# k-flouris/cmf

Hardware: AMD Instinct MI355X
Metric: log-density evals/sec (JtJ-cholesky path), MNIST D=784 d=64 bs=512 (higher is better)
Workload: dtype f32 (3x3 tangent convs as bf16x3 split MFMA, fp32 accumulate); 1 GPU; C3: MNIST-shaped (1,28,28) uint8-range + U[0,1) noise, non-square flow d=64, cholesky J^T J log-det + g_ij off-diagonal L1 + reconstruction, eval/no_grad; per_gpu_batch=512, global_batch=512, D=784, latent_dimension=64, parallelism=dp1

## Files before the change

### cmf_amd/_lib.py

```python
import ctypes as C
import os
import threading

_HERE = os.path.dirname(os.path.abspath(__file__))
LIB_PATH = os.path.join(_HERE, "libcmf_amd.so")

F_NONE, F_RELU, F_TANH, F_RAW, F_SELF_RELU, F_RELU_BITS = 0, 1, 2, 3, 4, 5
O_NONE, O_TANH, O_STANH = 0, 1, 2

_fp = C.c_void_p
_ll = C.c_longlong
_i = C.c_int
_f = C.c_float
_d = C.c_double


class ConvTangentArgs(C.Structure):
    _fields_ = [("x", _fp), ("x_np", _ll), ("x_ci", _ll), ("x_px", _ll),
                ("f", _fp), ("f_np", _ll), ("f_ci", _ll), ("f_px", _ll), ("fmode", _i),
                ("w", _fp),
                ("y", _fp), ("y_np", _ll), ("y_co", _ll), ("y_px", _ll),
                ("r", _fp), ("r_np", _ll), ("r_co", _ll), ("r_px", _ll),
                ("np", _i), ("cin", _i), ("cout", _i), ("H", _i), ("W", _i), ("nc", _i), ("taps", _i),
                ("bias", _fp), ("f_group", _i), ("x_sl", _ll), ("y_sl", _ll), ("r_sl", _ll),
                ("fo", _fp), ("fo_np", _ll), ("fo_co", _ll), ("fo_px", _ll), ("fomode", _i),
                ("mask_out", _fp), ("mask_np", _ll), ("amax_in", _fp), ("amax_out", _fp), ("live", _i)]


class ConvPrimalArgs(C.Structure):
    _fields_ = [("x", _fp), ("x_b", _ll), ("x_c", _ll), ("x_px", _ll),
                ("f", _fp), ("f_c", _ll), ("f_px", _ll), ("imode", _i),
                ("w", _fp), ("bias", _fp), ("sw", _fp), ("sb", _fp),
                ("y", _fp), ("y_b", _ll), ("y_c", _ll), ("y_px", _ll),
                ("g", _fp),
                ("r", _fp), ("r_b", _ll), ("r_c", _ll), ("r_px", _ll),
                ("omode", _i),
                ("B", _i), ("cin", _i), ("cout", _i), ("H", _i), ("W", _i), ("taps", _i)]


MLP_MAX_LAYERS = 8
WGRAD_MAX_BATCH = 16
# ... 166 lines not shown
```

### cmf_amd/csrc/conv_tangent.hip

```cpp
#include <type_traits>
#include "common.h"

namespace {

constexpr int CIC = 8;

template <int TAPS, int COT, int PXW>
struct Cfg {
  static constexpr int TW = 2 * PXW;
  static constexpr int TWH = TW + 2;
  static constexpr int PIXH = (TAPS == 9) ? 4 * TWH : 4 * PXW;
  static constexpr int XS_CI = PIXH * 16 + 16;
  static constexpr int WS_CI = (COT % 2) ? COT * 16 : COT * 16 + 16;
  static constexpr int XS_FLOATS = CIC * XS_CI;
  static constexpr int WS_FLOATS = TAPS * CIC * WS_CI;
  static constexpr int NX_ITEMS = CIC * PIXH * 4;
  static constexpr int NXIT = (NX_ITEMS + 255) / 256;
  static constexpr int NW_ITEMS = TAPS * CIC * COT * 4;
  static constexpr int NWIT = (NW_ITEMS + 255) / 256;
};

template <int TAPS, int COT, int PXW>
__global__ __launch_bounds__(256, 2) void conv_tangent_kernel(cmf_conv_tangent_args a, int tiles_x, int ntiles,
                                                                int nslices, int ncog, int cin_pad, int nsub) {
// ... 380 lines not shown

extern "C" int cmf_conv_tangent(const cmf_conv_tangent_args* ap, void* stream) {
  if (!ap) return CMF_EINVAL;
  const cmf_conv_tangent_args& a = *ap;
  if (!a.x || !a.w || !a.y || a.np <= 0 || a.cin <= 0 || a.cout <= 0 || a.H <= 0 || a.W <= 0) return CMF_EINVAL;
  if (a.taps != 1 && a.taps != 9) return CMF_EINVAL;
  if (a.nc <= 0 || a.nc % 16 || a.live) return CMF_EINVAL;
  if (a.fmode < CMF_F_NONE || a.fmode > CMF_F_SELF_RELU) return CMF_EINVAL;
  if (a.fmode != CMF_F_NONE && a.fmode != CMF_F_SELF_RELU && !a.f) return CMF_EINVAL;
  if ((a.x_np | a.x_ci | a.x_px | a.x_sl | a.y_sl | a.r_sl) % 4 || ((uintptr_t)a.x % 16) || ((uintptr_t)a.w % 16)) return CMF_EINVAL;
  if ((a.y_np | a.y_co | a.y_px) % 4 || ((uintptr_t)a.y % 16)) return CMF_EINVAL;
  if (a.r && ((a.r_np | a.r_co | a.r_px) % 4 || ((uintptr_t)a.r % 16))) return CMF_EINVAL;
  if (a.fo && (a.fomode < CMF_F_RELU || a.fomode > CMF_F_SELF_RELU)) return CMF_EINVAL;
  if (a.fo && a.fomode == CMF_F_SELF_RELU && ((a.fo_np | a.fo_co | a.fo_px) % 4 || (uintptr_t)a.fo % 16)) return CMF_EINVAL;
  if (a.mask_out && (a.cout % 16 || a.mask_np < (long long)a.H * a.W * (a.cout / 8))) return CMF_EINVAL;
  const long long HW = (long long)a.H * a.W;
  if (!fits_int((a.cin + 8) * a.x_ci + HW * a.x_px + a.nc) || !fits_int((a.cin + 8) * a.f_ci + HW * a.f_px) ||
      !fits_int((a.cout + 64) * a.y_co + HW * a.y_px + a.nc) || (a.r && !fits_int((a.cout + 64) * a.r_co + HW * a.r_px + a.nc)) ||
      HW > (1 << 24))
    return CMF_ERANGE;
  hipStream_t s = (hipStream_t)stream;
  if (thin_ok(a)) return launch_thin(a, s);
  const bool seven = (a.taps == 9) ? (a.W % 14 == 0) : (HW % 28 == 0 && HW % 32 != 0);
  if (a.taps == 9 && !seven && a.W % 8 == 0 && a.cout % 64 == 0) {
    const long long items8 = (long long)cmf_ceil_div(a.W, 16) * cmf_ceil_div(a.H, 2) * (a.nc / 16) * (a.cout / 64) * a.np;
    if (items8 * 4 <= 128) return launch_cot<9, 4>(a, s);
  }
  if (a.taps == 9) return seven ? launch_cot<9, 7>(a, s) : launch_cot<9, 8>(a, s);
  return seven ? launch_cot<1, 7>(a, s) : launch_cot<1, 8>(a, s);
}
// ... 1 lines not shown
```

### cmf_amd/csrc/conv_tangent_bf16x3.hip

```cpp
#include <cstdlib>
#include <type_traits>
#include "common.h"

#ifdef CMF_DBG_STAMP
__device__ unsigned long long cmf_dbg_stamps[3][64][4];
extern "C" int cmf_debug_read_stamps(void* out) {
  return (int)hipMemcpyFromSymbol(out, HIP_SYMBOL(cmf_dbg_stamps), sizeof(cmf_dbg_stamps));
}
#define STAMP(role, g, k)                                                                        \
  do {                                                                                            \
    if (blockIdx.x == 0 && (g) < 64 && lane == 0 && wave == ((role) == 1 ? 4 : 0)) {                   \
      unsigned long long t_;                                                                      \
      asm volatile("s_memtime %0\n\ts_waitcnt lgkmcnt(0)" : "=s"(t_)::"memory");                  \
      cmf_dbg_stamps[role][g][k] = t_;                                                            \
    }                                                                                             \
  } while (0)
__device__ unsigned long long cmf_dbg_wg_span[1024][2];
extern "C" int cmf_debug_read_wg_span(void* out) {
  return (int)hipMemcpyFromSymbol(out, HIP_SYMBOL(cmf_dbg_wg_span), sizeof(cmf_dbg_wg_span));
}
#define SPAN(k)                                                                                   \
  do {                                                                                            \
    if (lane == 0 && wave == 0 && blockIdx.x < 1024) {                                            \
      unsigned long long t_;                                                                      \
// ... 65 lines not shown
  return __builtin_bit_cast(float, (unsigned)(e + 127) << 23);
}

__device__ __forceinline__ int xslot(int col, int pix) { return (((col & 3) << 2) + (col >> 2) + ((pix & 1) << 2)) & 15; }

template <int COT, int PXW, int MODE, bool F16 = false, bool FRES = false, bool CKB = false>
__global__ __launch_bounds__(512, 2) void conv_tangent_bf16x3_kernel(cmf_conv_tangent_args a, int tiles_x, int ntiles,
                                                                       int nslices, int ncog, int total) {
  static_assert(!CKB || (!F16 && !FRES && (MODE == 1 || MODE == 3)), "checkerboard output: the forward tangent conv with a relu' factor");
  static_assert(!F16 || ((MODE == 2 || MODE == 4) && (COT == 4 || COT == 2)), "the fp16 variant is the primal pass: SELF mode (forward) or 4 (backward)");
  constexpr bool BWD = F16 && MODE == 4;
  static_assert(!BWD || FRES, "the backward form uses the epilogue with tile loads");
  constexpr bool HALF = F16 && COT == 2;
  constexpr int COG = HALF ? 32 : 64;
  static_assert(!FRES || F16, "residual-in-the-epilogue is the fp16 variant's");
  constexpr bool SELF = MODE == 2, RELU = MODE == 1, BITS = MODE == 3;
  constexpr bool PLAIN = !F16 && (MODE == 4 || MODE == 5);
  constexpr bool INPLACE = MODE == 5;
  constexpr bool NOF = SELF || PLAIN || BWD;
  constexpr int NF = NOF ? 0 : BITS ? 1 : 8;
  using C = BCfg<COT, PXW>;
  constexpr int CW = COT / 2, PW = CKB ? C::PW / 2 : C::PW;
  auto tp = [](int p) constexpr { return CKB ? 2 * p : p; };
  auto trow = [&](int p) constexpr { return tp(p) / C::TW; };
  static_assert(COT % 2 == 0, "the co-split wave layout needs an even number of output-channel tiles");
  extern __shared__ __attribute__((aligned(16))) unsigned char smem[];

  const int tid = threadIdx.x, lane = tid & 63;
  const int wave = __builtin_amdgcn_readfirstlane(tid >> 6);
  const bool loader = wave >= 4;
  SPAN(0);
// ... 48 lines not shown
#ifdef CMF_DBG_PRIO
    __builtin_amdgcn_s_setprio(3);
#endif
    const int lt = tid - 256;
    const int x_ci = (int)a.x_ci, x_px = (int)a.x_px, f_ci = (int)a.f_ci, f_px = (int)a.f_px;
    const int q = lt & 3, pix = lt >> 2;
    const int hy = pix / C::TWH, hx = pix % C::TWH;
    const float fc0 = (a.fmode == CMF_F_NONE || a.fmode == CMF_F_TANH || a.fmode == CMF_F_SELF_RELU) ? 1.f : 0.f;
    const float fc1 = (a.fmode == CMF_F_RELU) ? 1.f : 0.f;
    const float fc2 = (a.fmode == CMF_F_RAW) ? 1.f : 0.f;
    const float fc3 = (a.fmode == CMF_F_TANH) ? -1.f : 0.f;
    constexpr bool has_f = !NOF;
    const int fgrp = a.f_group > 1 ? a.f_group : 1;

    typedef int i32x4 __attribute__((ext_vector_type(4)));
    auto make_rsrc = [&](const void* p) {
      const unsigned long long u = reinterpret_cast<unsigned long long>(p);
      i32x4 d;
      d[0] = __builtin_amdgcn_readfirstlane((int)(unsigned)u);
      d[1] = __builtin_amdgcn_readfirstlane((int)((unsigned)(u >> 32) & 0xffffu));
      d[2] = -1;
      d[3] = 0x00020000;
      return d;
    };
    int cur_item = 0, cur_ch = 0;
    i32x4 xrs = make_rsrc(a.x), frs = xrs, wrs = make_rsrc(a.w);
    int xo = 0, fo = 0;
    float okf = 0.f;
    auto set_item = [&](int item) {
      int tile, slice, cog, np;
      decode(item, tile, slice, cog, np);
      const int y0 = C::TH * (tile / tiles_x), x0 = C::TW * (tile % tiles_x);
      xrs = make_rsrc(a.x + (long long)np * a.x_np + (long long)slice * (a.x_sl ? a.x_sl : 16));
      frs = BITS ? make_rsrc(reinterpret_cast<const unsigned char*>(a.f) + (long long)np * a.f_np)
                 : make_rsrc(a.f ? a.f + (long long)(np / fgrp) * a.f_np + (np % fgrp) : a.x);
      const int gy = y0 - 1 + hy, gx = x0 - 1 + hx;
      const bool ok = lt < C::NX_ITEMS && gy >= 0 && gy < a.H && gx >= 0 && gx < a.W;
      const int gpix = gy * a.W + gx;
      okf = ok ? 1.f : 0.f;
      xo = ok ? 4 * (gpix * x_px + q * 4) : 0;
      fo = ok ? (BITS ? gpix * (a.cin / 8) : 4 * (gpix * f_px)) : 0;
    };
    constexpr int NWOFF = COT == 4 ? 1 : C::NWIT;
    int woff[NWOFF];
    if (COT == 4) {
      woff[0] = lt << 4;
    } else {
#pragma unroll
      for (int it = 0; it < NWOFF; ++it) {
        int i = lt + 256 * it;
        i = i < C::NW_ITEMS ? i : C::NW_ITEMS - 1;
        const int rest = i & 63, t = i >> 6;
        const int cot = t % COT, s = (t / COT) % 3, hl = t / (3 * COT);
        woff[it] = (((hl * 3 + s) * 4 + cot) * 64 + rest) << 4;
      }
    }
// ... 24 lines not shown
        if (COT == 4 && it % 3 == 2) {
          asm volatile("s_nop 4\n\tbuffer_load_dwordx4 %0, %1, %2, %3 offen" : "=&v"(wreg[it]) : "v"(vo), "s"(wrs2), "s"(so) : "memory");
          continue;
        }
        asm volatile("s_nop 4\n\tbuffer_load_dwordx4 %0, %1, %2, %3 offen" : "=&v"(wreg[it]) : "v"(vo), "s"(wrs), "s"(so) : "memory");
      }
      if (++wcur_ch == nchunks) {
        wcur_ch = 0;
        if (wcur_item + 1 < n_items) wset_item(++wcur_item);
        else wcur_ch = nchunks - 1;
      }
    };
#pragma unroll
    for (int j = 0; j < 8; ++j) r0.f[j] = r1.f[j] = r2.f[j] = 0.f;

    auto prefetch = [&](Regs& r) {
      const int ch = cur_ch;
      {
        const int s0 = 4 * (ch * 8 + 0) * x_ci, s1 = 4 * (ch * 8 + 1) * x_ci, s2 = 4 * (ch * 8 + 2) * x_ci,
                  s3 = 4 * (ch * 8 + 3) * x_ci, s4 = 4 * (ch * 8 + 4) * x_ci, s5 = 4 * (ch * 8 + 5) * x_ci,
                  s6 = 4 * (ch * 8 + 6) * x_ci, s7 = 4 * (ch * 8 + 7) * x_ci;
        asm volatile(
            "s_nop 4\n\t"
            "buffer_load_dwordx4 %0, %8, %9, %10 offen\n\t"
            "buffer_load_dwordx4 %1, %8, %9, %11 offen\n\t"
            "buffer_load_dwordx4 %2, %8, %9, %12 offen\n\t"
            "buffer_load_dwordx4 %3, %8, %9, %13 offen\n\t"
            "buffer_load_dwordx4 %4, %8, %9, %14 offen\n\t"
            "buffer_load_dwordx4 %5, %8, %9, %15 offen\n\t"
            "buffer_load_dwordx4 %6, %8, %9, %16 offen\n\t"
            "buffer_load_dwordx4 %7, %8, %9, %17 offen"
            : "=&v"(r.x[0]), "=&v"(r.x[1]), "=&v"(r.x[2]), "=&v"(r.x[3]), "=&v"(r.x[4]), "=&v"(r.x[5]), "=&v"(r.x[6]),
              "=&v"(r.x[7])
            : "v"(xo), "s"(xrs), "s"(s0), "s"(s1), "s"(s2), "s"(s3), "s"(s4), "s"(s5), "s"(s6), "s"(s7)
            : "memory");
      }
      if constexpr (BITS) {
        asm volatile("s_nop 4\n\tbuffer_load_ubyte %0, %1, %2, %3 offen" : "=&v"(r.f[0]) : "v"(fo), "s"(frs), "s"(ch) : "memory");
      } else if (has_f) {
        const int s0 = 4 * (ch * 8 + 0) * f_ci, s1 = 4 * (ch * 8 + 1) * f_ci, s2 = 4 * (ch * 8 + 2) * f_ci,
                  s3 = 4 * (ch * 8 + 3) * f_ci, s4 = 4 * (ch * 8 + 4) * f_ci, s5 = 4 * (ch * 8 + 5) * f_ci,
                  s6 = 4 * (ch * 8 + 6) * f_ci, s7 = 4 * (ch * 8 + 7) * f_ci;
        asm volatile(
            "s_nop 4\n\t"
            "buffer_load_dword %0, %8, %9, %10 offen\n\t"
            "buffer_load_dword %1, %8, %9, %11 offen\n\t"
            "buffer_load_dword %2, %8, %9, %12 offen\n\t"
            "buffer_load_dword %3, %8, %9, %13 offen\n\t"
            "buffer_load_dword %4, %8, %9, %14 offen\n\t"
            "buffer_load_dword %5, %8, %9, %15 offen\n\t"
            "buffer_load_dword %6, %8, %9, %16 offen\n\t"
            "buffer_load_dword %7, %8, %9, %17 offen"
            : "=&v"(r.f[0]), "=&v"(r.f[1]), "=&v"(r.f[2]), "=&v"(r.f[3]), "=&v"(r.f[4]), "=&v"(r.f[5]), "=&v"(r.f[6]),
// ... 58 lines not shown
        for (int c = 0; c < 4; ++c) {
          u32x4 h;
#pragma unroll
          for (int jj = 0; jj < 4; ++jj)
            h[jj] = __builtin_amdgcn_perm(__builtin_bit_cast(unsigned, r.x[2 * jj + 1][c]),
                                          __builtin_bit_cast(unsigned, r.x[2 * jj][c]), 0x07060302u);
          const int off = ((pix * 16 + xslot(q * 4 + c, pix)) << 4);
          *reinterpret_cast<u32x4*>(Xh + off) = h;
          *reinterpret_cast<u32x4*>(Xl + off) = h;
        }
#else
        float v[8][4];
#pragma unroll
        for (int j = 0; j < 8; ++j) {
          const float f = r.f[j];
          const float m = NOF ? (F16 ? r.okf * xscale : r.okf) : BITS ? (((__builtin_bit_cast(unsigned, r.f[0]) >> j) & 1u) ? r.okf : 0.f)
                               : RELU ? (f > 0.f ? r.okf : 0.f)
                                              : r.okf * (fc0 + fc1 * (f > 0.f ? 1.f : 0.f) + f * (fc2 + fc3 * f));
#pragma unroll
          for (int c = 0; c < 4; ++c) v[j][c] = (SELF ? fmaxf(r.x[j][c], 0.f) : r.x[j][c]) * m;
        }
#pragma unroll
        for (int c = 0; c < 4; ++c) {
          u32x4 h, l;
#pragma unroll
          for (int jj = 0; jj < 4; ++jj) {
            const float e = v[2 * jj][c], o = v[2 * jj + 1][c];
            if constexpr (F16) {
              unsigned lo_;
              h[jj] = split_f16(e, o, lo_);
              l[jj] = lo_;
            } else {
              const unsigned hb = pack_lo(e, o);
              const float re = e - __builtin_bit_cast(float, hb << 16);
              const float ro = o - __builtin_bit_cast(float, hb & 0xffff0000u);
// ... 15 lines not shown
      for (int it = 0; it < C::NWIT; ++it) {
        const int i = lt + 256 * it;
        if (COT == 4 && it % 3 == 2 && !wquad) continue;
        if (i < C::NW_ITEMS) {
          const int rest = i & 63, t = i >> 6;
          const int cot = t % COT, s = (t / COT) % 3, hl = t / (3 * COT);
          unsigned char* dst = (hl ? Wl : Wh) + ((((s * COT + cot) * 64) + rest) << 4);
          *reinterpret_cast<u32x4*>(dst) = wreg[it];
        }
      }
    };

    if (n_items > 0) {
      set_item(0);
      wset_item(0);
      prefetch(r0);
      prefetch(r1);
      prefetch(r2);
      prefetch_w();
      STAMP2(4, 10, 0);
      asm volatile("s_waitcnt vmcnt(0)" ::: "memory");
      STAMP2(4, 10, 1);
      wait_x(r0);
      commit(r0, 0);
      prefetch_w();
      STAMP2(4, 10, 2);
    }
    __syncthreads();
    auto iter = [&](int g, Regs& freed, Regs& next) {
      STAMP(1, g, 0);
// ... 139 lines not shown
  i32x4 nxt_rrs = r_rsrc(np_, slice_, cog_, n_items > 0);
  auto init_pixel = [&](const Item& it, const i32x4& rrs_in, int p) __attribute__((always_inline)) {
    i32x4 rrs;
#pragma unroll
    for (int i = 0; i < 4; ++i) rrs[i] = __builtin_amdgcn_readfirstlane(rrs_in[i]);
#pragma unroll
    for (int c = 0; c < CW; ++c) {
      const int so = it.rpix + 4 * ((trow(p) * a.W + tp(p) % C::TW + (CKB ? ck_o[trow(p) & 1] : 0)) * r_px + c * 16 * r_co);
      asm volatile("s_nop 4\n\tbuffer_load_dwordx4 %0, %1, %2, %3 offen" : "=v"(acc[p][c]) : "v"(rvoff), "s"(rrs), "s"(so) : "memory");
    }
  };
  unsigned omask[PW];
  const bool use_omask = PLAIN && a.fomode == CMF_F_RELU_BITS;
  constexpr bool inplace = INPLACE;
  auto load_omask = [&](const Item& it) __attribute__((always_inline)) {
    if constexpr (PLAIN) {
      const unsigned long long base = reinterpret_cast<unsigned long long>(a.fo) + (unsigned long long)it.np * a.fo_np +
                                      (unsigned)(it.cog * 8 + cohalf * 4);
      const unsigned lo = __builtin_amdgcn_readfirstlane((int)(unsigned)base);
      const unsigned hi = __builtin_amdgcn_readfirstlane((int)(unsigned)(base >> 32));
      const unsigned long long sb = ((unsigned long long)hi << 32) | lo;
      const int stride = a.cout / 8;
#pragma unroll
      for (int p = 0; p < PW; ++p) {
        const int off = __builtin_amdgcn_readfirstlane((it.pix0 + (p / C::TW) * a.W + p % C::TW) * stride);
        unsigned w;
        asm volatile("s_load_dword %0, %1, %2\n\ts_waitcnt lgkmcnt(0)" : "=&s"(w) : "s"(sb), "s"(off) : "memory");
        omask[p] = use_omask ? w : ~0u;
      }
    }
  };
  auto store_pixel = [&](const Item& it, int p, f32x4 radd0, f32x4 radd1, f32x4 m0 = f32x4{}, f32x4 m1 = f32x4{}) __attribute__((always_inline)) {
    [[maybe_unused]] unsigned mbits = 0;
    [[maybe_unused]] f32x4 vst[CW];
#pragma unroll
    for (int c = 0; c < CW; ++c) {
      f32x4 v = acc[p][c];
      int vo = yvoff;
      if constexpr (PLAIN) {
        const bool on = (omask[p] >> (c * 16 + cl)) & 1u;
        if constexpr (inplace) vo = on ? yvoff : Y_DROP;
        else v = on ? v : f32x4{0.f, 0.f, 0.f, 0.f};
      }
      if constexpr (BWD) {
        v = v * oscale;
        const f32x4 mm = c == 0 ? m0 : m1;
#pragma unroll
        for (int r = 0; r < 4; ++r) v[r] = mm[r] > 0.f ? v[r] : 0.f;
      } else if constexpr (HALF) v = v * oscale + ((it.cog & 1) ? bias_h1 : bias[c]);
      else if constexpr (F16) v = v * oscale + bias[c];
      else v += bias[c];
      if constexpr (FRES) v += c == 0 ? radd0 : radd1;
      __builtin_amdgcn_raw_buffer_store_b128(__builtin_bit_cast(bu32x4, v), cur_yrs, vo,
                                             it.ypix + 4 * ((CKB ? trow(p) * (a.W / 2) + tp(p) % C::TW / 2 : (p / C::TW) * a.W + p % C::TW) * y_px +
                                                            c * 16 * y_co), 0);
      if constexpr (F16) {
        vst[c] = v;
        if constexpr (BWD)
// ... 349 lines not shown
  auto k = conv_tangent_bf16x3_kernel<COT, PXW, MODE, F16, FRES, CKB>;
  constexpr int lds = C::LDS_BYTES;
  if (hipError_t e = cmf_set_dynamic_lds((const void*)k, lds); e != hipSuccess) return (int)e;
  const int n_cu = cmf_device_cus();
  int grid = (int)(total < n_cu ? total : n_cu);
#ifdef CMF_DBG_STAMP
  if (const char* e = getenv("CMF_DBG_GRID")) grid = atoi(e) < grid ? atoi(e) : grid;
#endif
  hipLaunchKernelGGL(k, dim3(grid), dim3(512), lds, s, a, tiles_x, tiles, nslices, ncog, (int)total);
  CMF_LAUNCH_CHECK();
  return 0;
}

template <int PXW>
int launch_cot(const cmf_conv_tangent_args& a, hipStream_t s) {
  if (a.fmode == CMF_F_SELF_RELU) return (a.cout > 32) ? launch<4, PXW, 2>(a, s) : launch<2, PXW, 2>(a, s);
  if (a.fmode == CMF_F_RELU) return (a.cout > 32) ? launch<4, PXW, 1>(a, s) : launch<2, PXW, 1>(a, s);
  if (a.fmode == CMF_F_RELU_BITS) return (a.cout > 32) ? launch<4, PXW, 3>(a, s) : launch<2, PXW, 3>(a, s);
  if (a.fmode == CMF_F_NONE && a.fomode == CMF_F_RELU_BITS && a.r) {
    return launch<4, PXW, 5>(a, s);
  }
  if (a.fmode == CMF_F_NONE) return (a.cout > 32) ? launch<4, PXW, 4>(a, s) : launch<2, PXW, 4>(a, s);
  return (a.cout > 32) ? launch<4, PXW, 0>(a, s) : launch<2, PXW, 0>(a, s);
}

inline bool fits_int(long long v) { return v >= 0 && v < (1LL << 29); }

}

extern "C" int cmf_pack_weight_bf16x3_t(const float* w, void* out, int cout, int cin, int transpose, long long* out_bytes, void* stream);
// ... 30 lines not shown
extern "C" int cmf_conv_tangent_bf16x3(const cmf_conv_tangent_args* ap, void* stream) {
  if (!ap) return CMF_EINVAL;
  const cmf_conv_tangent_args& a = *ap;
  if (!a.x || !a.w || !a.y || a.np <= 0 || a.cin <= 0 || a.cout <= 0 || a.H <= 0 || a.W <= 0) return CMF_EINVAL;
  if (a.taps != 9 || a.cin % 32 || a.nc <= 0 || a.nc % 16) return CMF_EINVAL;
  if (a.fmode < CMF_F_NONE || a.fmode > CMF_F_RELU_BITS) return CMF_EINVAL;
  if (a.fmode != CMF_F_SELF_RELU && a.fmode != CMF_F_NONE && !a.f) return CMF_EINVAL;
  if (a.mask_out) return CMF_EINVAL;
  if (a.fo) {
    const bool inplace = a.r == a.y && a.r_np == a.y_np && a.r_co == a.y_co && a.r_px == a.y_px && a.r_sl == a.y_sl;
    if (a.fmode != CMF_F_NONE || a.fomode != CMF_F_RELU_BITS || (a.r && !inplace) || a.cout % 64) return CMF_EINVAL;
    if (a.r && a.bias) return CMF_EINVAL;
    if (a.fo_np % 4 || (uintptr_t)a.fo % 4 || a.fo_np < (long long)a.H * a.W * (a.cout / 8)) return CMF_EINVAL;
  }
  if (a.fmode == CMF_F_RELU_BITS && a.f_np < (long long)a.H * a.W * (a.cin / 8)) return CMF_EINVAL;
  if ((a.x_np | a.x_ci | a.x_px | a.x_sl | a.y_sl | a.r_sl) % 4 || ((uintptr_t)a.x % 16) || ((uintptr_t)a.w % 16)) return CMF_EINVAL;
  if ((a.y_np | a.y_co | a.y_px) % 4 || ((uintptr_t)a.y % 16)) return CMF_EINVAL;
  if (a.r && ((a.r_np | a.r_co | a.r_px) % 4 || ((uintptr_t)a.r % 16))) return CMF_EINVAL;
  const long long HW = (long long)a.H * a.W;
  if (!fits_int((a.cin + 8) * a.x_ci + HW * a.x_px + a.nc) || !fits_int((a.cin + 8) * a.f_ci + HW * a.f_px) ||
      !fits_int((a.cout + 64) * a.y_co + HW * a.y_px + a.nc + 64) ||
      (a.r && !fits_int((a.cout + 64) * a.r_co + HW * a.r_px + a.nc)) ||
      HW > (1 << 24))
    return CMF_ERANGE;
  hipStream_t s = (hipStream_t)stream;
  const bool t14 = a.W % 14 == 0 && a.H % 2 == 0, t8 = a.W % 8 == 0 && a.H % 4 == 0;
  if (!(t14 || t8) || !(a.cout % 64 == 0 || a.cout == 32)) return CMF_EINVAL;
  if (a.bias && a.cout > 64) return CMF_EINVAL;
  if (a.live) {
    if (a.live < 0 || a.live > 2 || (a.fmode != CMF_F_RELU && a.fmode != CMF_F_RELU_BITS) || a.fo || a.bias || a.cout % 64 || a.W % 2)
// ... 7 lines not shown
    b.fo_np = 0;
    b.fomode = CMF_F_NONE;
    return t14 ? launch_cot<7>(b, s) : launch_cot<4>(b, s);
  }
  return t14 ? launch_cot<7>(a, s) : launch_cot<4>(a, s);
}

extern "C" int cmf_conv_tangent_f16x3(const cmf_conv_tangent_args* ap, void* stream) {
  return cmf_conv_tangent_f16x3_item(ap, 0, stream);
}

extern "C" int cmf_conv_tangent_f16x3_item(const cmf_conv_tangent_args* ap, int item_channels, void* stream) {
  if (!ap || (item_channels != 0 && item_channels != 32 && item_channels != 64)) return CMF_EINVAL;
  const cmf_conv_tangent_args& a = *ap;
  if (!a.x || !a.w || !a.y || a.np <= 0 || a.cin <= 0 || a.cout <= 0 || a.H <= 0 || a.W <= 0) return CMF_EINVAL;
  if (a.taps != 9 || a.cin % 32 || a.nc <= 0 || a.nc % 16 || a.cout % 64 || a.live) return CMF_EINVAL;
  const bool bwd = a.fmode == CMF_F_NONE && a.fo && a.fomode == CMF_F_SELF_RELU;
  if (!bwd && (a.fmode != CMF_F_SELF_RELU || a.fo)) return CMF_EINVAL;
  if (bwd && (a.bias || a.mask_out || (a.fo_np | a.fo_co | a.fo_px) % 4 || (uintptr_t)a.fo % 16)) return CMF_EINVAL;
  if (a.mask_out && (a.mask_np % 4 || (uintptr_t)a.mask_out % 4 || a.mask_np < (long long)a.H * a.W * (a.cout / 8) ||
                     16 * a.mask_np >= 0x7fffff00LL))
    return CMF_EINVAL;
  if ((a.x_np | a.x_ci | a.x_px | a.x_sl | a.y_sl | a.r_sl) % 4 || ((uintptr_t)a.x % 16) || ((uintptr_t)a.w % 16)) return CMF_EINVAL;
  if ((a.y_np | a.y_co | a.y_px) % 4 || ((uintptr_t)a.y % 16)) return CMF_EINVAL;
  if (a.r && ((a.r_np | a.r_co | a.r_px) % 4 || ((uintptr_t)a.r % 16))) return CMF_EINVAL;
  const long long HW = (long long)a.H * a.W;
  if (!fits_int((a.cin + 8) * a.x_ci + HW * a.x_px + a.nc) || !fits_int((a.cout + 64) * a.y_co + HW * a.y_px + a.nc + 64) ||
      (a.r && !fits_int((a.cout + 64) * a.r_co + HW * a.r_px + a.nc)) ||
      (bwd && !fits_int((a.cout + 64) * a.fo_co + HW * a.fo_px + a.nc)) || HW > (1 << 24))
    return CMF_ERANGE;
  const bool t14 = a.W % 14 == 0 && a.H % 2 == 0, t8 = a.W % 8 == 0 && a.H % 4 == 0;
// ... 18 lines not shown
```

### cmf_amd/engine.py

```python
import ctypes as C
import threading

import numpy as np
import torch
import torch.nn as nn

from . import _lib
from ._lib import (F_NONE, F_RELU, F_TANH, F_RAW, F_SELF_RELU, F_RELU_BITS, O_NONE, O_TANH, O_STANH, ConvPrimalArgs,
                   ConvTangentArgs)


def _stream():
    return C.c_void_p(torch.cuda.current_stream().cuda_stream)


def _p(t):
    return None if t is None else C.c_void_p(t.data_ptr())


def require_gpu(t, what="input"):
    if not t.is_cuda:
        raise RuntimeError(f"cmf_amd: {what} is on {t.device}; the log-density path runs only through the HIP "
                           "kernels on an AMD GPU (there is no CPU fallback)")
    if t.dtype != torch.float32:
# ... 285 lines not shown
    a = ConvPrimalArgs()
    a.x = C.c_void_p(x_ptr_t.data_ptr() + 4 * int(x_off)); a.x_b, a.x_c, a.x_px = int(x_b), int(x_c), int(x_px)
    a.f = _p(mask); a.f_c, a.f_px = int(f_c), int(f_px); a.imode = imode
    a.w = _p(PACKS.get(weight, taps)); a.bias = _p(bias); a.sw = _p(sw); a.sb = _p(sb)
    a.y = _p(y); a.y_b, a.y_c, a.y_px = int(y_b), int(y_c), int(y_px)
    a.g = _p(g)
    a.r = _p(res); a.r_b, a.r_c, a.r_px = int(y_b), int(y_c), int(y_px)
    a.omode = omode
    a.B, a.cin, a.cout, a.H, a.W, a.taps = int(B), int(cin), int(cout), int(H), int(W), int(taps)
    _lib.check(lib.cmf_conv_primal(C.byref(a), _stream()), "cmf_conv_primal")


def conv_tangent(x_t, x_off, x_np, x_ci, x_px, weight, taps, y_t, y_np, y_co, y_px, np_, cin, cout, H, W, nc,
                 fmode=F_NONE, f=None, f_np=0, f_ci=0, f_px=0, res_t=None, transpose=False, bias=None, f_group=1,
                 x_sl=16, y_sl=16, precision=None, y_off=0, res_off=0, fo=None, fo_np=0, fo_co=0, fo_px=0, fomode=F_NONE,
                 mask_out=None, mask_np=0, amax_in=None, amax_out=None, item_channels=0, live=0, res_np=None):
    lib = _lib.load()
    a = ConvTangentArgs()
    a.x = C.c_void_p(x_t.data_ptr() + 4 * int(x_off)); a.x_np, a.x_ci, a.x_px = int(x_np), int(x_ci), int(x_px)
    a.f = _p(f); a.f_np, a.f_ci, a.f_px = int(f_np), int(f_ci), int(f_px); a.fmode = fmode
    obits = isinstance(fo, BitMask)
    inplace = res_t is not None and res_t.data_ptr() == y_t.data_ptr() and int(res_off) == int(y_off)
    precision = precision or cfg().tangent
    split = (precision == "bf16x3" and _shape_ok_bf16x3(taps, cin, W, transpose, H, cout)
             and not (bias is not None and cout > 64)
             and ((fmode != F_NONE and fo is None) or
                  (fmode == F_NONE and (fo is None or (obits and (res_t is None or inplace) and cout % 64 == 0)))))
    pbwd = fmode == F_NONE and fo is not None and not obits and fomode == F_SELF_RELU
    f16 = (precision == "f16x3" and cout % 64 == 0 and _shape_ok_bf16x3(taps, cin, W, transpose, H, cout)
           and not (bias is not None and cout > 64)
           and ((fmode == F_SELF_RELU and fo is None and not transpose) or (pbwd and bias is None and mask_out is None)))
    assert not obits or split, "bit-mask output factors are applied by the split-precision kernel only"
    if obits:
        fo, fo_np, fo_co, fo_px, fomode = fo.data, fo.np_bytes, 0, 0, F_RELU_BITS
    a.w = _p(PACKS.get(weight, taps, transpose, bf16x3="f16x3" if f16 else split))
    a.y = C.c_void_p(y_t.data_ptr() + 4 * int(y_off)); a.y_np, a.y_co, a.y_px = int(y_np), int(y_co), int(y_px)
    a.r = None if res_t is None else C.c_void_p(res_t.data_ptr() + 4 * int(res_off))
    a.r_np, a.r_co, a.r_px = int(y_np if res_np is None else res_np), int(y_co), int(y_px)
    a.fo = _p(fo); a.fo_np, a.fo_co, a.fo_px, a.fomode = int(fo_np), int(fo_co), int(fo_px), int(fomode)
    a.mask_out = _p(mask_out); a.mask_np = int(mask_np)
    assert not (fmode == F_RELU_BITS and not split), "bit-mask factors are read by the split-precision kernel only"
    assert not (mask_out is not None and split), "sign bits are written by the fp32 and the fp16-split kernels only"
    a.amax_in, a.amax_out = (_p(amax_in), _p(amax_out)) if f16 else (None, None)
    a.live = int(live)
    assert not live or split, "checkerboard output is the split-precision kernel's"
    a.np, a.cin, a.cout, a.H, a.W, a.nc, a.taps = int(np_), int(cin), int(cout), int(H), int(W), int(nc), int(taps)
    a.bias = _p(bias); a.f_group = int(f_group)
    a.x_sl, a.y_sl, a.r_sl = int(x_sl), int(y_sl), int(y_sl)
    fn, what = ((lib.cmf_conv_tangent_f16x3, "cmf_conv_tangent_f16x3") if f16 else
                (lib.cmf_conv_tangent_bf16x3, "cmf_conv_tangent_bf16x3") if split else (lib.cmf_conv_tangent, "cmf_conv_tangent"))
    launch = lambda: _lib.check(fn(C.byref(a), _stream()), what)
    if f16 and item_channels:
        launch = lambda: _lib.check(lib.cmf_conv_tangent_f16x3_item(C.byref(a), int(item_channels), _stream()), "cmf_conv_tangent_f16x3_item")
    if fmode == F_SELF_RELU and not f16 and _lib.tracing():
        run = launch

        def launch():
            with _lib.role("primal"):
                run()
    TIMER = _timer()
# ... 783 lines not shown

def _view_rows(T, view):
    if T.layout == "panel":
        HW = view.geom.HW
        rows = T.data[: T.B * T.N * T.nc].view(T.B, T.N // HW, HW * T.nc)[:, view.chan_off::view.chan_step][:, :view.cin]
        out = Tangent(T.B, view.cin * HW, T.nc, "panel", T.data.device)
    else:
        rows = T.data[: T.B * T.N * T.nc].view(T.N, T.B * T.nc)[view.chan_off::view.chan_step][:view.cin]
        out = Tangent(T.B, view.cin, T.nc, "fmajor", T.data.device)
    out.data.view(rows.shape).copy_(rows)
    return out


CHECKERBOARD_TAIL = True


def net_tangent(net, T, view, acts, transpose_packs=False, save=None):
    geo, B, nc, dev = view.geom, T.B, T.nc, T.data.device
    if save is not None:
        save.append(_view_rows(T, view))
    if net.kind == "resnet":
        conv0, blocks, convf = _resnet_parts(net)
        hid, cout, H, W, HW = conv0.out_channels, convf.out_channels, geo.H, geo.W, geo.HW
        new = lambda c: Tangent(B, c * HW, nc, "panel", dev)
        pn = lambda c: (c * HW * nc, HW * nc, nc)
        hd = (hid * HW * nc, 16, hid * nc)
        hsl = hid * 16
        h = new(hid)
        conv_tangent(T.data, view.chan_off * HW * nc, T.t_b, view.chan_step * HW * nc, nc, conv0.weight, 9, h.data, *hd,
                     B, view.cin, hid, H, W, nc, fmode=F_RAW if view.mask is not None else F_NONE, f=view.mask, f_np=0,
                     f_ci=HW, f_px=1, y_sl=hsl)
        fg = getattr(acts, "f_group", 1)
        fs = dict(f_np=hid * HW * fg, f_ci=HW * fg, f_px=fg, f_group=fg)
        fk = lambda t: dict(fmode=F_RELU_BITS, f=t.data, f_np=t.np_bytes) if isinstance(t, BitMask) else dict(fmode=F_RELU, f=t, **fs)
        u, h2 = new(hid), new(hid)
        compact = (CHECKERBOARD_TAIL and view.live is not None and save is None and fg == 1 and len(blocks) > 0 and hid % 64 == 0
                   and W % 2 == 0 and _use_bf16x3(9, hid, W, False, H, hid))
        for k, blk in enumerate(blocks):
            a_in, c1 = acts[2 * k], acts[2 * k + 1]
            conv_tangent(h.data, 0, *hd, blk.conv1.weight, 9, u.data, *hd, B, hid, hid, H, W, nc, x_sl=hsl, y_sl=hsl, **fk(a_in))
            if compact and k + 1 == len(blocks):
                HWc = HW // 2
                hc = Tangent(B, hid * HWc, nc, "panel", dev)
                conv_tangent(u.data, 0, *hd, blk.conv2.weight, 9, hc.data, hid * HWc * nc, 16, hid * nc, B, hid, hid, H, W, nc,
                             res_t=h.data, res_np=hd[0], x_sl=hsl, y_sl=hsl, live=view.live["parity"], **fk(c1))
                a_last = gather_primal(acts[-1], view.live["act_idx"], hid * HWc)
                yt = Tangent(B, cout * HWc, nc, "panel", dev)
                conv_tangent(hc.data, 0, hid * HWc * nc, 16, hid * nc, convf.weight, 1, yt.data, cout * HWc * nc, HWc * nc, nc, B, hid,
                             cout, H, W // 2, nc, fmode=F_RELU, f=a_last, x_sl=hsl, f_np=hid * HWc, f_ci=HWc, f_px=1)
                yt.compact = True
                return yt
            conv_tangent(u.data, 0, *hd, blk.conv2.weight, 9, h2.data, *hd, B, hid, hid, H, W, nc, res_t=h.data, x_sl=hsl,
                         y_sl=hsl, **fk(c1))
            if save is not None:
                save += [h, u]
# ... 257 lines not shown
```

### include/cmf_amd.h

```cpp
#ifndef CMF_AMD_H
#define CMF_AMD_H

#ifdef __cplusplus
extern "C" {
#endif

#define CMF_EINVAL (-1)
#define CMF_ERANGE (-2)

#define CMF_F_NONE 0
#define CMF_F_RELU 1
#define CMF_F_TANH 2
#define CMF_F_RAW  3
#define CMF_F_SELF_RELU 4
#define CMF_F_RELU_BITS 5

#define CMF_O_NONE  0
#define CMF_O_TANH  1
#define CMF_O_STANH 2

const char* cmf_version(void);

int cmf_pack_weight(const float* w, float* out, int cout, int cin, int taps, int transpose,
                    long long* out_floats, void* stream);
// ... 7 lines not shown
typedef struct {
  const float* x; long long x_np, x_ci, x_px;
  const float* f; long long f_np, f_ci, f_px;
  int fmode;
  const float* w;
  float* y;       long long y_np, y_co, y_px;
  const float* r; long long r_np, r_co, r_px;
  int np, cin, cout, H, W, nc, taps;
  const float* bias;
  int f_group;
  long long x_sl, y_sl, r_sl;
  const float* fo; long long fo_np, fo_co, fo_px; int fomode;
  void* mask_out; long long mask_np;
  const float* amax_in; float* amax_out;
  int live;
} cmf_conv_tangent_args;
int cmf_conv_tangent(const cmf_conv_tangent_args* a, void* stream);

int cmf_pack_weight_bf16x3(const float* w, void* out, int cout, int cin, long long* out_bytes, void* stream);
int cmf_pack_weight_bf16x3_t(const float* w, void* out, int cout, int cin, int transpose, long long* out_bytes, void* stream);
int cmf_conv_tangent_bf16x3(const cmf_conv_tangent_args* a, void* stream);

int cmf_pack_weight_f16x3(const float* w, void* out, int cout, int cin, int transpose, long long* out_bytes, void* stream);
int cmf_conv_tangent_f16x3(const cmf_conv_tangent_args* a, void* stream);
int cmf_conv_tangent_f16x3_item(const cmf_conv_tangent_args* a, int item_channels, void* stream);
int cmf_absmax(const float* x, long long n, float* out, void* stream);

long long cmf_conv_tangent_wgrad_ws(const cmf_conv_tangent_args* a);
int cmf_conv_tangent_wgrad(const cmf_conv_tangent_args* a, const float* gy, float* dw, float* ws, long long ws_bytes,
                           void* stream);
// ... 138 lines not shown
```

Baseline: 1419 evals/s.

## Skip dead-ReLU loads and stores in bf16x3 tangent conv via bitmasks

Adds a ymask store filter to the split-precision tangent conv. Output lanes whose next-layer ReLU mask bit is zero are sent to a dropped address, since the following conv would zero them anyway. In the RELU_BITS mode, input loads for masked-off channels are redirected out of range through buffer-descriptor record limits, replacing the per-element multiply by the mask. The mask bytes are now prefetched one stage ahead with their own item cursor. This trades memory traffic for extra scalar mask loads and per-element address selects, and it relies on dead entries never being read unmasked downstream.

```diff
diff --git a/cmf_amd/_lib.py b/cmf_amd/_lib.py
--- a/cmf_amd/_lib.py
+++ b/cmf_amd/_lib.py
@@ -24,7 +24,8 @@
                 ("np", _i), ("cin", _i), ("cout", _i), ("H", _i), ("W", _i), ("nc", _i), ("taps", _i),
                 ("bias", _fp), ("f_group", _i), ("x_sl", _ll), ("y_sl", _ll), ("r_sl", _ll),
                 ("fo", _fp), ("fo_np", _ll), ("fo_co", _ll), ("fo_px", _ll), ("fomode", _i),
-                ("mask_out", _fp), ("mask_np", _ll), ("amax_in", _fp), ("amax_out", _fp), ("live", _i)]
+                ("mask_out", _fp), ("mask_np", _ll), ("amax_in", _fp), ("amax_out", _fp), ("live", _i),
+                ("ymask", _fp), ("ymask_np", _ll)]
 
 
 class ConvPrimalArgs(C.Structure):
diff --git a/cmf_amd/csrc/conv_tangent.hip b/cmf_amd/csrc/conv_tangent.hip
--- a/cmf_amd/csrc/conv_tangent.hip
+++ b/cmf_amd/csrc/conv_tangent.hip
@@ -418,6 +418,7 @@
   if (a.fo && (a.fomode < CMF_F_RELU || a.fomode > CMF_F_SELF_RELU)) return CMF_EINVAL;
   if (a.fo && a.fomode == CMF_F_SELF_RELU && ((a.fo_np | a.fo_co | a.fo_px) % 4 || (uintptr_t)a.fo % 16)) return CMF_EINVAL;
   if (a.mask_out && (a.cout % 16 || a.mask_np < (long long)a.H * a.W * (a.cout / 8))) return CMF_EINVAL;
+  if (a.ymask) return CMF_EINVAL;
   const long long HW = (long long)a.H * a.W;
   if (!fits_int((a.cin + 8) * a.x_ci + HW * a.x_px + a.nc) || !fits_int((a.cin + 8) * a.f_ci + HW * a.f_px) ||
       !fits_int((a.cout + 64) * a.y_co + HW * a.y_px + a.nc) || (a.r && !fits_int((a.cout + 64) * a.r_co + HW * a.r_px + a.nc)) ||
diff --git a/cmf_amd/csrc/conv_tangent_bf16x3.hip b/cmf_amd/csrc/conv_tangent_bf16x3.hip
--- a/cmf_amd/csrc/conv_tangent_bf16x3.hip
+++ b/cmf_amd/csrc/conv_tangent_bf16x3.hip
@@ -103,7 +103,9 @@
   constexpr bool HALF = F16 && COT == 2;
   constexpr int COG = HALF ? 32 : 64;
   static_assert(!FRES || F16, "residual-in-the-epilogue is the fp16 variant's");
-  constexpr bool SELF = MODE == 2, RELU = MODE == 1, BITS = MODE == 3;
+  constexpr bool YMASK = !F16 && (MODE == 6 || MODE == 7);
+  static_assert(!YMASK || (COT == 4 && !CKB), "the store filter: whole 64-channel groups, every pixel");
+  constexpr bool SELF = MODE == 2, RELU = MODE == 1 || MODE == 6, BITS = MODE == 3 || MODE == 7;
   constexpr bool PLAIN = !F16 && (MODE == 4 || MODE == 5);
   constexpr bool INPLACE = MODE == 5;
   constexpr bool NOF = SELF || PLAIN || BWD;
@@ -182,12 +184,13 @@
     const int fgrp = a.f_group > 1 ? a.f_group : 1;
 
     typedef int i32x4 __attribute__((ext_vector_type(4)));
-    auto make_rsrc = [&](const void* p) {
+    constexpr int X_RECORDS = BITS ? 0x7fffff00 : -1, X_DROP = 0x7ffffff0;
+    auto make_rsrc = [&](const void* p, int records = -1) {
       const unsigned long long u = reinterpret_cast<unsigned long long>(p);
       i32x4 d;
       d[0] = __builtin_amdgcn_readfirstlane((int)(unsigned)u);
       d[1] = __builtin_amdgcn_readfirstlane((int)((unsigned)(u >> 32) & 0xffffu));
-      d[2] = -1;
+      d[2] = records;
       d[3] = 0x00020000;
       return d;
     };
@@ -195,19 +198,28 @@
     i32x4 xrs = make_rsrc(a.x), frs = xrs, wrs = make_rsrc(a.w);
     int xo = 0, fo = 0;
     float okf = 0.f;
+    [[maybe_unused]] int mcur_item = 0, mcur_ch = 0, mo = 0;
+    [[maybe_unused]] auto mset_item = [&](int item) {
+      int tile, slice, cog, np;
+      decode(item, tile, slice, cog, np);
+      const int y0 = C::TH * (tile / tiles_x), x0 = C::TW * (tile % tiles_x);
+      frs = make_rsrc(reinterpret_cast<const unsigned char*>(a.f) + (long long)np * a.f_np, X_RECORDS);
+      const int gy = y0 - 1 + hy, gx = x0 - 1 + hx;
+      const bool ok = lt < C::NX_ITEMS && gy >= 0 && gy < a.H && gx >= 0 && gx < a.W;
+      mo = ok ? (gy * a.W + gx) * (a.cin / 8) : X_DROP;
+    };
     auto set_item = [&](int item) {
       int tile, slice, cog, np;
       decode(item, tile, slice, cog, np);
       const int y0 = C::TH * (tile / tiles_x), x0 = C::TW * (tile % tiles_x);
-      xrs = make_rsrc(a.x + (long long)np * a.x_np + (long long)slice * (a.x_sl ? a.x_sl : 16));
-      frs = BITS ? make_rsrc(reinterpret_cast<const unsigned char*>(a.f) + (long long)np * a.f_np)
-                 : make_rsrc(a.f ? a.f + (long long)(np / fgrp) * a.f_np + (np % fgrp) : a.x);
+      xrs = make_rsrc(a.x + (long long)np * a.x_np + (long long)slice * (a.x_sl ? a.x_sl : 16), X_RECORDS);
+      if constexpr (!BITS) frs = make_rsrc(a.f ? a.f + (long long)(np / fgrp) * a.f_np + (np % fgrp) : a.x);
       const int gy = y0 - 1 + hy, gx = x0 - 1 + hx;
       const bool ok = lt < C::NX_ITEMS && gy >= 0 && gy < a.H && gx >= 0 && gx < a.W;
       const int gpix = gy * a.W + gx;
       okf = ok ? 1.f : 0.f;
       xo = ok ? 4 * (gpix * x_px + q * 4) : 0;
-      fo = ok ? (BITS ? gpix * (a.cin / 8) : 4 * (gpix * f_px)) : 0;
+      fo = ok ? 4 * (gpix * f_px) : 0;
     };
     constexpr int NWOFF = COT == 4 ? 1 : C::NWIT;
     int woff[NWOFF];
@@ -262,9 +274,43 @@
 #pragma unroll
     for (int j = 0; j < 8; ++j) r0.f[j] = r1.f[j] = r2.f[j] = 0.f;
 
+    [[maybe_unused]] auto prefetch_mask = [&](Regs& r) {
+      asm volatile("s_nop 4\n\tbuffer_load_ubyte %0, %1, %2, %3 offen" : "=&v"(r.f[0]) : "v"(mo), "s"(frs), "s"(mcur_ch) : "memory");
+      if (++mcur_ch == nchunks) {
+        mcur_ch = 0;
+        if (mcur_item + 1 < n_items) mset_item(++mcur_item);
+        else mcur_ch = nchunks - 1;
+      }
+    };
     auto prefetch = [&](Regs& r) {
       const int ch = cur_ch;
-      {
+      if constexpr (BITS) {
+        const int s0 = 4 * (ch * 8 + 0) * x_ci, s1 = 4 * (ch * 8 + 1) * x_ci, s2 = 4 * (ch * 8 + 2) * x_ci,
+                  s3 = 4 * (ch * 8 + 3) * x_ci, s4 = 4 * (ch * 8 + 4) * x_ci, s5 = 4 * (ch * 8 + 5) * x_ci,
+                  s6 = 4 * (ch * 8 + 6) * x_ci, s7 = 4 * (ch * 8 + 7) * x_ci;
+        const unsigned mb = __builtin_bit_cast(unsigned, r.f[0]);
+        int o[8];
+#pragma unroll
+        for (int j = 0; j < 8; ++j) {
+          const int t = __builtin_amdgcn_sbfe(mb, j, 1);
+          o[j] = (xo & t) | (X_DROP & ~t);
+        }
+        asm volatile(
+            "s_nop 4\n\t"
+            "buffer_load_dwordx4 %0, %8, %16, %17 offen\n\t"
+            "buffer_load_dwordx4 %1, %9, %16, %18 offen\n\t"
+            "buffer_load_dwordx4 %2, %10, %16, %19 offen\n\t"
+            "buffer_load_dwordx4 %3, %11, %16, %20 offen\n\t"
+            "buffer_load_dwordx4 %4, %12, %16, %21 offen\n\t"
+            "buffer_load_dwordx4 %5, %13, %16, %22 offen\n\t"
+            "buffer_load_dwordx4 %6, %14, %16, %23 offen\n\t"
+            "buffer_load_dwordx4 %7, %15, %16, %24 offen"
+            : "=&v"(r.x[0]), "=&v"(r.x[1]), "=&v"(r.x[2]), "=&v"(r.x[3]), "=&v"(r.x[4]), "=&v"(r.x[5]), "=&v"(r.x[6]),
+              "=&v"(r.x[7])
+            : "v"(o[0]), "v"(o[1]), "v"(o[2]), "v"(o[3]), "v"(o[4]), "v"(o[5]), "v"(o[6]), "v"(o[7]), "s"(xrs), "s"(s0), "s"(s1),
+              "s"(s2), "s"(s3), "s"(s4), "s"(s5), "s"(s6), "s"(s7)
+            : "memory");
+      } else {
         const int s0 = 4 * (ch * 8 + 0) * x_ci, s1 = 4 * (ch * 8 + 1) * x_ci, s2 = 4 * (ch * 8 + 2) * x_ci,
                   s3 = 4 * (ch * 8 + 3) * x_ci, s4 = 4 * (ch * 8 + 4) * x_ci, s5 = 4 * (ch * 8 + 5) * x_ci,
                   s6 = 4 * (ch * 8 + 6) * x_ci, s7 = 4 * (ch * 8 + 7) * x_ci;
@@ -284,7 +330,7 @@
             : "memory");
       }
       if constexpr (BITS) {
-        asm volatile("s_nop 4\n\tbuffer_load_ubyte %0, %1, %2, %3 offen" : "=&v"(r.f[0]) : "v"(fo), "s"(frs), "s"(ch) : "memory");
+        prefetch_mask(r);
       } else if (has_f) {
         const int s0 = 4 * (ch * 8 + 0) * f_ci, s1 = 4 * (ch * 8 + 1) * f_ci, s2 = 4 * (ch * 8 + 2) * f_ci,
                   s3 = 4 * (ch * 8 + 3) * f_ci, s4 = 4 * (ch * 8 + 4) * f_ci, s5 = 4 * (ch * 8 + 5) * f_ci,
@@ -373,11 +419,11 @@
 #pragma unroll
         for (int j = 0; j < 8; ++j) {
           const float f = r.f[j];
-          const float m = NOF ? (F16 ? r.okf * xscale : r.okf) : BITS ? (((__builtin_bit_cast(unsigned, r.f[0]) >> j) & 1u) ? r.okf : 0.f)
+          const float m = NOF ? (F16 ? r.okf * xscale : r.okf) : BITS ? 1.f
                                : RELU ? (f > 0.f ? r.okf : 0.f)
                                               : r.okf * (fc0 + fc1 * (f > 0.f ? 1.f : 0.f) + f * (fc2 + fc3 * f));
 #pragma unroll
-          for (int c = 0; c < 4; ++c) v[j][c] = (SELF ? fmaxf(r.x[j][c], 0.f) : r.x[j][c]) * m;
+          for (int c = 0; c < 4; ++c) v[j][c] = BITS ? r.x[j][c] : (SELF ? fmaxf(r.x[j][c], 0.f) : r.x[j][c]) * m;
         }
 #pragma unroll
         for (int c = 0; c < 4; ++c) {
@@ -423,6 +469,13 @@
     if (n_items > 0) {
       set_item(0);
       wset_item(0);
+      if constexpr (BITS) {
+        mset_item(0);
+        prefetch_mask(r0);
+        prefetch_mask(r1);
+        prefetch_mask(r2);
+        asm volatile("s_waitcnt vmcnt(0)" : "+v"(r0.f[0]), "+v"(r1.f[0]), "+v"(r2.f[0])::"memory");
+      }
       prefetch(r0);
       prefetch(r1);
       prefetch(r2);
@@ -592,8 +645,9 @@
   const bool use_omask = PLAIN && a.fomode == CMF_F_RELU_BITS;
   constexpr bool inplace = INPLACE;
   auto load_omask = [&](const Item& it) __attribute__((always_inline)) {
-    if constexpr (PLAIN) {
-      const unsigned long long base = reinterpret_cast<unsigned long long>(a.fo) + (unsigned long long)it.np * a.fo_np +
+    if constexpr (PLAIN || YMASK) {
+      const unsigned long long base = (YMASK ? reinterpret_cast<unsigned long long>(a.ymask) + (unsigned long long)it.np * a.ymask_np
+                                             : reinterpret_cast<unsigned long long>(a.fo) + (unsigned long long)it.np * a.fo_np) +
                                       (unsigned)(it.cog * 8 + cohalf * 4);
       const unsigned lo = __builtin_amdgcn_readfirstlane((int)(unsigned)base);
       const unsigned hi = __builtin_amdgcn_readfirstlane((int)(unsigned)(base >> 32));
@@ -604,7 +658,7 @@
         const int off = __builtin_amdgcn_readfirstlane((it.pix0 + (p / C::TW) * a.W + p % C::TW) * stride);
         unsigned w;
         asm volatile("s_load_dword %0, %1, %2\n\ts_waitcnt lgkmcnt(0)" : "=&s"(w) : "s"(sb), "s"(off) : "memory");
-        omask[p] = use_omask ? w : ~0u;
+        omask[p] = (YMASK || use_omask) ? w : ~0u;
       }
     }
   };
@@ -620,6 +674,7 @@
         if constexpr (inplace) vo = on ? yvoff : Y_DROP;
         else v = on ? v : f32x4{0.f, 0.f, 0.f, 0.f};
       }
+      if constexpr (YMASK) vo = ((omask[p] >> (c * 16 + cl)) & 1u) ? yvoff : Y_DROP;
       if constexpr (BWD) {
         v = v * oscale;
         const f32x4 mm = c == 0 ? m0 : m1;
@@ -999,6 +1054,7 @@
 
 template <int PXW>
 int launch_cot(const cmf_conv_tangent_args& a, hipStream_t s) {
+  if (a.ymask) return a.fmode == CMF_F_RELU ? launch<4, PXW, 6>(a, s) : launch<4, PXW, 7>(a, s);
   if (a.fmode == CMF_F_SELF_RELU) return (a.cout > 32) ? launch<4, PXW, 2>(a, s) : launch<2, PXW, 2>(a, s);
   if (a.fmode == CMF_F_RELU) return (a.cout > 32) ? launch<4, PXW, 1>(a, s) : launch<2, PXW, 1>(a, s);
   if (a.fmode == CMF_F_RELU_BITS) return (a.cout > 32) ? launch<4, PXW, 3>(a, s) : launch<2, PXW, 3>(a, s);
@@ -1059,6 +1115,10 @@
     if (a.fo_np % 4 || (uintptr_t)a.fo % 4 || a.fo_np < (long long)a.H * a.W * (a.cout / 8)) return CMF_EINVAL;
   }
   if (a.fmode == CMF_F_RELU_BITS && a.f_np < (long long)a.H * a.W * (a.cin / 8)) return CMF_EINVAL;
+  if (a.ymask) {
+    if ((a.fmode != CMF_F_RELU && a.fmode != CMF_F_RELU_BITS) || a.cout % 64 || a.live || a.fo || a.r || a.bias) return CMF_EINVAL;
+    if (a.ymask_np % 4 || (uintptr_t)a.ymask % 4 || a.ymask_np < (long long)a.H * a.W * (a.cout / 8)) return CMF_EINVAL;
+  }
   if ((a.x_np | a.x_ci | a.x_px | a.x_sl | a.y_sl | a.r_sl) % 4 || ((uintptr_t)a.x % 16) || ((uintptr_t)a.w % 16)) return CMF_EINVAL;
   if ((a.y_np | a.y_co | a.y_px) % 4 || ((uintptr_t)a.y % 16)) return CMF_EINVAL;
   if (a.r && ((a.r_np | a.r_co | a.r_px) % 4 || ((uintptr_t)a.r % 16))) return CMF_EINVAL;
@@ -1096,7 +1156,7 @@
   if (!ap || (item_channels != 0 && item_channels != 32 && item_channels != 64)) return CMF_EINVAL;
   const cmf_conv_tangent_args& a = *ap;
   if (!a.x || !a.w || !a.y || a.np <= 0 || a.cin <= 0 || a.cout <= 0 || a.H <= 0 || a.W <= 0) return CMF_EINVAL;
-  if (a.taps != 9 || a.cin % 32 || a.nc <= 0 || a.nc % 16 || a.cout % 64 || a.live) return CMF_EINVAL;
+  if (a.taps != 9 || a.cin % 32 || a.nc <= 0 || a.nc % 16 || a.cout % 64 || a.live || a.ymask) return CMF_EINVAL;
   const bool bwd = a.fmode == CMF_F_NONE && a.fo && a.fomode == CMF_F_SELF_RELU;
   if (!bwd && (a.fmode != CMF_F_SELF_RELU || a.fo)) return CMF_EINVAL;
   if (bwd && (a.bias || a.mask_out || (a.fo_np | a.fo_co | a.fo_px) % 4 || (uintptr_t)a.fo % 16)) return CMF_EINVAL;
diff --git a/cmf_amd/engine.py b/cmf_amd/engine.py
--- a/cmf_amd/engine.py
+++ b/cmf_amd/engine.py
@@ -323,7 +323,7 @@
 def conv_tangent(x_t, x_off, x_np, x_ci, x_px, weight, taps, y_t, y_np, y_co, y_px, np_, cin, cout, H, W, nc,
                  fmode=F_NONE, f=None, f_np=0, f_ci=0, f_px=0, res_t=None, transpose=False, bias=None, f_group=1,
                  x_sl=16, y_sl=16, precision=None, y_off=0, res_off=0, fo=None, fo_np=0, fo_co=0, fo_px=0, fomode=F_NONE,
-                 mask_out=None, mask_np=0, amax_in=None, amax_out=None, item_channels=0, live=0, res_np=None):
+                 mask_out=None, mask_np=0, amax_in=None, amax_out=None, item_channels=0, live=0, res_np=None, ymask=None):
     lib = _lib.load()
     a = ConvTangentArgs()
     a.x = C.c_void_p(x_t.data_ptr() + 4 * int(x_off)); a.x_np, a.x_ci, a.x_px = int(x_np), int(x_ci), int(x_px)
@@ -353,6 +353,9 @@
     a.amax_in, a.amax_out = (_p(amax_in), _p(amax_out)) if f16 else (None, None)
     a.live = int(live)
     assert not live or split, "checkerboard output is the split-precision kernel's"
+    assert ymask is None or split, "the store filter is the split-precision kernel's"
+    if ymask is not None:
+        a.ymask, a.ymask_np = _p(ymask.data), int(ymask.np_bytes)
     a.np, a.cin, a.cout, a.H, a.W, a.nc, a.taps = int(np_), int(cin), int(cout), int(H), int(W), int(nc), int(taps)
     a.bias = _p(bias); a.f_group = int(f_group)
     a.x_sl, a.y_sl, a.r_sl = int(x_sl), int(y_sl), int(y_sl)
@@ -1166,6 +1169,8 @@
 
 CHECKERBOARD_TAIL = True
 
+SKIP_DEAD_ROWS = True
+
 
 def net_tangent(net, T, view, acts, transpose_packs=False, save=None):
     geo, B, nc, dev = view.geom, T.B, T.nc, T.data.device
@@ -1188,9 +1193,11 @@
         u, h2 = new(hid), new(hid)
         compact = (CHECKERBOARD_TAIL and view.live is not None and save is None and fg == 1 and len(blocks) > 0 and hid % 64 == 0
                    and W % 2 == 0 and _use_bf16x3(9, hid, W, False, H, hid))
+        filt = SKIP_DEAD_ROWS and save is None and hid % 64 == 0 and _use_bf16x3(9, hid, W, False, H, hid)
         for k, blk in enumerate(blocks):
             a_in, c1 = acts[2 * k], acts[2 * k + 1]
-            conv_tangent(h.data, 0, *hd, blk.conv1.weight, 9, u.data, *hd, B, hid, hid, H, W, nc, x_sl=hsl, y_sl=hsl, **fk(a_in))
+            conv_tangent(h.data, 0, *hd, blk.conv1.weight, 9, u.data, *hd, B, hid, hid, H, W, nc, x_sl=hsl, y_sl=hsl, **fk(a_in),
+                         ymask=c1 if filt and isinstance(c1, BitMask) else None)
             if compact and k + 1 == len(blocks):
                 HWc = HW // 2
                 hc = Tangent(B, hid * HWc, nc, "panel", dev)
diff --git a/include/cmf_amd.h b/include/cmf_amd.h
--- a/include/cmf_amd.h
+++ b/include/cmf_amd.h
@@ -45,6 +45,7 @@
   void* mask_out; long long mask_np;
   const float* amax_in; float* amax_out;
   int live;
+  const void* ymask; long long ymask_np;
 } cmf_conv_tangent_args;
 int cmf_conv_tangent(const cmf_conv_tangent_args* a, void* stream);
 
```

Measured after the change: 1475 evals/s (median of 6 runs). +3.9%, better.
